# nyenyu12/BioInformatics-project-for-Shotgun-Metagenomics-Pseudo-alignment-shotgun-

Hardware: AMD Instinct MI355X
Metric: reads/sec pseudo-aligned (k=31, 150bp) at 1/2/4/8 GPUs; % HBM roofline (higher is better)
Workload: dtype u8

## Files before the change

bioinformatics-project-for-shotgun-metagenomics-pseudo-alignment-shotgun-_amd/csrc/pa_align.hip:

```cpp
#include <hip/hip_runtime.h>

#include <algorithm>
#include <cstdio>
#include <cstdlib>
#include <cstring>
#include <type_traits>
#include <vector>

#include "pa_device.h"
#include "pa_internal.h"

using namespace pad;

namespace {

constexpr int kBlock = 256;
constexpr int kWaves = kBlock / 64;
constexpr uint32_t kSegMaxWaves = 16384;
constexpr uint32_t kSegSlackWaves = 8192, kSegSlackChunks = 5;
constexpr uint64_t kSegSlack = 64ull * kSegSlackChunks * kSegSlackWaves;
constexpr uint32_t kLdsGenomeCap = 2048;

enum : uint32_t { F_MRQ = 1, F_MKQ = 2, F_MG = 4 };

// ... 15 lines not shown
    uint64_t nb_base1, nb_split;
    const uint32_t *nbbig_ld;
    uint64_t nbbig_mask;
    int nb_spec;
    const uint32_t *tile_nbbig;
    const uint4 *tile_nbm;
    int mg_nb;
    const uint32_t *gblk;
    const uint64_t *bloom;
    const uint64_t *tile_rcp;
    const uint32_t *mm_bits;
    uint32_t mm_lg;
    const uint32_t *tile_rcnb;
    uint32_t bloom_lg;
    int walk_rounds;
    int tpos_local;
    uint32_t lane_maxpend;
    int lane_noanchor;
    int dbg_mode;
    const uint8_t *seq;
    const uint8_t *qual;
    const uint64_t *off;
    uint64_t n;
    uint64_t base;
    pa::DevParams prm;
    unsigned long long *stats;
    unsigned long long *uniq;
    unsigned long long *amb;
    unsigned long long *first;
    uint32_t *queue;
    unsigned long long *qcount;
    unsigned long long *deferred_total;
    uint32_t *queue_hard;
    unsigned long long *queue_hard_count;
    uint32_t *queue_na;
    unsigned long long *queue_na_count;
    uint64_t *queue_na_keys;
    uint32_t *queue_rc;
    uint64_t *queue_rc_anc;
    unsigned long long *queue_rc_count;
    uint32_t *queue_na2;
    unsigned long long *queue_na2_count;
    uint64_t na_min;
    uint32_t na_seg;
    uint32_t *seg_cnt;
    uint32_t nseg;
    uint64_t seg_cap;
    uint64_t queue_cap;
    uint32_t *lane_next;
    const uint4 *qmask;
    const uint8_t *qdrop;
    const uint32_t *rlist;
    const unsigned long long *rlist_count;
    unsigned long long *dbg;
    uint8_t *as_type;
    uint32_t *as_len, *as_g, *as_qf, *as_hr;
};

__device__ __forceinline__ uint64_t first_key(uint64_t read, uint32_t rank) { return (read << 20) | rank; }


struct WgCounters {
    uint32_t *uniq;
    uint32_t *amb;
    unsigned long long *first;
    bool lds;
};

__device__ __forceinline__ void count_genome(const AlignArgs &a, const WgCounters &c, uint32_t g, bool unique,
                                             uint32_t times, uint64_t key) {
    if (c.lds) {
        atomicAdd(unique ? &c.uniq[g] : &c.amb[g], times);
        if (key < c.first[g]) atomicMin(&c.first[g], (unsigned long long)key);
    } else {
        atomicAdd(unique ? &a.uniq[g] : &a.amb[g], (unsigned long long)times);
        atomicMin(&a.first[g], (unsigned long long)key);
    }
}

#include "pa_fast.h"

constexpr int kQmDwords = 44;
template <int KQ>
__device__ __forceinline__ void quality_read(const uint8_t *__restrict__ qual, uint64_t o, uint32_t len, int k,
                                             uint32_t T, int64_t mrq, uint32_t flags, uint4 &mask, uint8_t &drop) {
    typedef uint32_t u32x4_a4 __attribute__((ext_vector_type(4), aligned(4)));
    const u32x4_a4 *sp = (const u32x4_a4 *)(qual + (o & ~3ull));
    const uint32_t sb = 8 * (uint32_t)(o & 3);
    uint32_t dw[kQmDwords + 4];
#pragma unroll
    for (int c = 0; c < (kQmDwords + 4) / 4; c++) {
        const u32x4_a4 v = sp[c];
        dw[4 * c] = v.x, dw[4 * c + 1] = v.y, dw[4 * c + 2] = v.z, dw[4 * c + 3] = v.w;
    }
    uint32_t rd[kQmDwords];
#pragma unroll
    for (int j = 0; j < kQmDwords; j++) rd[j] = __builtin_amdgcn_alignbit(dw[j + 1], dw[j], sb);
    const uint32_t nfull = len >> 2, pmask = (len & 3) ? (1u << (8 * (len & 3))) - 1 : 0u;
    uint32_t run_tot = 0, total = 0, part = 0;
#pragma unroll
    for (int j = 0; j < kQmDwords; j++) {
        const bool at = (uint32_t)j == nfull;
        total = at ? run_tot : total;
        part = at ? rd[j] : part;
        run_tot = __builtin_amdgcn_sad_u8(rd[j], 0u, run_tot);
    }
// ... 470 lines not shown
                    const uint32_t i = atomicAdd(&n_rank, 1u);
                    if (i < kRankLds) rank_key[i] = ld_agent(&ws.g_specmin[g]);
                }
                __syncthreads();
                for (uint32_t t = threadIdx.x; t < nt; t += kBlock) {
                    const uint32_t g = ws.touched[t];
                    if (ld_agent(&ws.g_spec[g]) == 0) continue;
                    const uint32_t mw = ld_agent(&ws.g_specmin[g]);
                    uint32_t rank = 0;
                    if (nspec <= kRankLds) {
                        for (uint32_t u = 0; u < nspec; u++) rank += rank_key[u] < mw;
                    } else {
                        for (uint32_t u = 0; u < nt; u++) {
                            const uint32_t h = ws.touched[u];
                            if (ld_agent(&ws.g_spec[h]) > 0 && ld_agent(&ws.g_specmin[h]) < mw) rank++;
                        }
                    }
                    if (x.detail == 2) x.lists[x.list_off[r] + rank] = g;
                    if (!x.detail) {
                        atomicAdd(&a.amb[g], 1ull);
                        atomicMin(&a.first[g], (unsigned long long)first_key(read_idx, rank));
                    }
                }
            }
            __syncthreads();
            for (uint32_t t = threadIdx.x; t < nt; t += kBlock) {
                const uint32_t g = ws.touched[t];
                st_agent(&ws.g_spec[g], 0u);
                st_agent(&ws.g_specmin[g], NONE);
                st_agent(&ws.g_tot[g], 0u);
                st_agent(&ws.g_totmin[g], NONE);
            }
            __syncthreads();
            if (threadIdx.x == 0) n_touched = n_cls = 0;
            __syncthreads();
        }
        if (threadIdx.x == 0) {
            if (x.detail) {
                x.type_out[r] = type;
                x.qf_out[r] = qf;
                x.hr_out[r] = hr;
                x.len_out[r] = list_len;
            } else {
                atomicAdd(&a.stats[type == PA_UNMAPPED ? 2 : (type == PA_UNIQUELY_MAPPED ? 0 : 1)], 1ull);
                if (has_mkq && qf) atomicAdd(&a.stats[4], (unsigned long long)qf);
                if (has_mg && hr) atomicAdd(&a.stats[5], (unsigned long long)hr);
            }
        }
        __syncthreads();
    }
}


size_t fast_lds_bytes(uint32_t G, int wpl, bool need_q) {
    size_t cnt = G <= kLdsGenomeCap ? (((size_t)((G + 1) & ~1u) * 16 + 15) / 16 * 16) : 0;
    size_t wl = wpl == 1 ? fast_wave_bytes<1>(need_q) : wpl == 2 ? fast_wave_bytes<2>(need_q) : fast_wave_bytes<4>(need_q);
    return cnt + kWaves * wl;
}

const char *env(const char *name) { return std::getenv(name); }
bool env_is(const char *name, char c) { const char *e = env(name); return e && e[0] == c; }
uint64_t env_u64(const char *name, uint64_t unset) { const char *e = env(name); return e ? std::strtoull(e, nullptr, 10) : unset; }
int env_int(const char *name, int unset) { const char *e = env(name); return e ? std::atoi(e) : unset; }
int env_01(const char *name) { const char *e = env(name); return e ? e[0] == '1' : -1; }

struct Switches {
    bool no_qelide = env("PA_NO_QELIDE");
    bool no_lane = env_is("PA_NO_LANE", '1');
    uint64_t lane_grid = env_u64("PA_LANE_GRID", ~0ull);
    uint32_t lane_maxpend = (uint32_t)env_int("PA_LANE_MAXPEND", 96);
    int lane_noanchor = env_01("PA_LANE_NOANCHOR");
    uint64_t na_min = env_u64("PA_NA_MIN", 32768);
    bool na_seg = !env_is("PA_NA_SEG", '0');
    bool na_rcwalk = !env_is("PA_NA_RCWALK", '0');
    bool na_rcnb = !env_is("PA_NA_RCNB", '0');
    bool mm_bits = !env_is("PA_MM_BITS", '0');
    bool no_nbbig = env("PA_NO_NBBIG");
    bool no_nbm = env("PA_NO_NBM");
    bool no_mgnb = env("PA_NO_MGNB");
    int walk_rounds = env_int("PA_WALK_ROUNDS", 1);
    int dbg_mode = env_int("PA_DBG_MODE", 0);
};

template <int N> using int_c = std::integral_constant<int, N>;

template <int N0, int... Ns, class F>
auto with_int(int n, F &&f) {
    if constexpr (sizeof...(Ns) == 0) return f(int_c<N0>{});
    else return n == N0 ? f(int_c<N0>{}) : with_int<Ns...>(n, f);
}

template <class F>
auto with_filters(uint32_t flags, F &&f) {
    const auto with_mg = [&](auto need_q, auto win_q) {
        return (flags & F_MG) ? f(need_q, win_q, std::true_type{}) : f(need_q, win_q, std::false_type{});
    };
    if (flags & F_MKQ) return with_mg(std::true_type{}, std::true_type{});
    if (flags & F_MRQ) return with_mg(std::true_type{}, std::false_type{});
    return with_mg(std::false_type{}, std::false_type{});
}

template <bool WIN_Q, class F>
auto with_shape(int nw, bool nm4, F &&f) {
    return with_int<3, 2, 1>(nw, [&](auto w) {
        if constexpr (!WIN_Q && w() == 1)
            if (nm4) return f(int_c<4>{}, w);
        return f(int_c<2>{}, w);
    });
}

using AlignKernel = void (*)(AlignArgs);
pa_status resident_grid(AlignKernel kern, int block, size_t shm, uint64_t want, unsigned &grid) {
    if (shm > 64 * 1024) PA_HIP(hipFuncSetAttribute((const void *)kern, hipFuncAttributeMaxDynamicSharedMemorySize, (int)shm));
    int per_cu = 0, dev = 0, cus = 256;
    PA_HIP(hipOccupancyMaxActiveBlocksPerMultiprocessor(&per_cu, kern, block, shm));
    PA_HIP(hipGetDevice(&dev));
    PA_HIP(hipDeviceGetAttribute(&cus, hipDeviceAttributeMultiprocessorCount, dev));
    const uint64_t resident = (uint64_t)std::max(1, per_cu) * (uint64_t)cus;
    grid = (unsigned)std::max<uint64_t>(1, std::min<uint64_t>(want, resident));
    return PA_OK;
}

struct KernelTimer {
    pa_index *idx;
    hipStream_t st;
    int slot;
    hipEvent_t e0 = nullptr;
    KernelTimer(pa_index *i, hipStream_t s, int sl) : idx(i), st(s), slot(sl) {
        if (idx && idx->profile && hipEventCreate(&e0) == hipSuccess) hipEventRecord(e0, st);
    }
    ~KernelTimer() {
        hipEvent_t e1 = nullptr;
        if (e0 && hipEventCreate(&e1) == hipSuccess && hipEventRecord(e1, st) == hipSuccess)
            idx->kev.push_back({slot, e0, e1});
        else if (e0)
            hipEventDestroy(e0);
    }
};

pa_status launch_timed(pa_index *prof, int slot, AlignKernel kern, unsigned grid, size_t shm, hipStream_t st,
                       const AlignArgs &a) {
    KernelTimer kt(prof, st, slot);
    hipLaunchKernelGGL(kern, dim3(grid), dim3(kBlock), shm, st, a);
    PA_HIP(hipGetLastError());
    return PA_OK;
}

pa_status launch_wave(const AlignArgs &a, pa_index *prof, int nw, int wpl, hipStream_t st) {
    const size_t shm = fast_lds_bytes(a.G, wpl, (a.prm.flags & (F_MRQ | F_MKQ)) != 0);
    const bool dense = a.G <= 64;
    const AlignKernel kern = with_int<1, 2, 3, 4>(nw, [&](auto w) {
        constexpr int NW = w();
        return with_int<1, 2, 4>(wpl, [&](auto l) -> AlignKernel {
            return dense ? k_align_fast<NW, l(), true> : k_align_fast<NW, l(), false>;
        });
    });
    unsigned grid = 0;
    PA_TRY(resident_grid(kern, kBlock, shm, (a.n + kWaves - 1) / kWaves, grid));
    return launch_timed(prof, PA_PROF_WAVE, kern, grid, shm, st, a);
}

constexpr uint64_t kRcnbMinReads = 32768;
struct LaneKernels { AlignKernel lane, rc, na; };
template <bool AS>
pa_status launch_lane(const AlignArgs &a0, const Switches &sw, hipStream_t st, pa_index *prof, bool long_reads, int nw) {
    const bool win_q = (a0.prm.flags & F_MKQ) != 0;
    const bool mg = (a0.prm.flags & F_MG) != 0;
    const bool nm4 = long_reads && !win_q && nw == 1;
    AlignArgs a = a0;
    const size_t shm = lane_lds_bytes(a.G, nm4 ? 4 : 2, lane_sched(win_q, mg, nm4 ? 4 : 2, nw));
    const LaneKernels kern = with_filters(a.prm.flags, [&](auto nq, auto wq, auto g) {
        constexpr bool NEED_Q = nq(), WIN_Q = wq(), MG = g();
        return LaneKernels{
            with_shape<WIN_Q>(nw, nm4, [](auto nm, auto w) -> AlignKernel { return k_align_lane<NEED_Q, WIN_Q, MG, nm(), w(), AS>; }),
            k_align_lane_rc<NEED_Q, WIN_Q, MG, AS>,
            with_int<3, 2, 1>(nw, [](auto w) -> AlignKernel {
                if constexpr (w() == 1) return k_align_lane_na<NEED_Q, WIN_Q, MG, AS>;
                else return k_align_lane_naw<NEED_Q, WIN_Q, MG, w(), AS>;
            })};
    });
    const uint64_t want = (a.n + kBlock - 1) / kBlock;
    unsigned grid = 0;
    PA_TRY(resident_grid(kern.lane, kBlock, shm, want, grid));
    grid = (unsigned)std::max<uint64_t>(1, std::min<uint64_t>(grid, sw.lane_grid));
    const uint64_t waves = (uint64_t)grid * kWaves, chunks = (a.n + 63) / 64;
    a.nseg = (uint32_t)waves;
    a.seg_cap = 64 * ((chunks + waves - 1) / waves + kLaneClaimHeld);
    a.na_seg = a.queue_na && a.queue_na_keys && a.seg_cnt && !nm4 && nw == 1 && waves <= kSegMaxWaves &&
               waves * a.seg_cap <= a.queue_cap && sw.na_seg;
    PA_TRY(launch_timed(prof, PA_PROF_LANE, kern.lane, grid, shm, st, a));
    if (!a.queue_na) return PA_OK;
    AlignArgs b = a;
    if (prof && prof->rcnb_pending && a.queue_na_keys) {
        unsigned long long c = 0;
        PA_HIP(hipMemcpyAsync(&c, a.queue_na_count, 8, hipMemcpyDeviceToHost, st));
        PA_HIP(hipStreamSynchronize(st));
        if (c >= std::max<uint64_t>(kRcnbMinReads, a.n / 64)) {
            PA_TRY(pa::index_build_rcnb(prof, st));
            if (sw.na_rcnb) b.tile_rcnb = prof->tile_rcnb;
        } else if (++prof->rcnb_checks >= 2) {
            prof->rcnb_pending = 0;
        }
    }
    if (a.queue_na_keys) {
        const unsigned sgrid = a.na_seg ? (a.nseg + kSegGroup - 1) / kSegGroup
                                        : (unsigned)std::max<uint64_t>(1, std::min<uint64_t>(
                                              (a.n + kBlock * 4 - 1) / (kBlock * 4), 8192));
        PA_TRY(launch_timed(prof, PA_PROF_RC_SEEDS, k_rc_seeds, sgrid, 0, st, b));
        PA_TRY(resident_grid(kern.rc, kBlock, 0, want, grid));
        PA_TRY(launch_timed(prof, PA_PROF_LANE_RC, kern.rc, grid, 0, st, b));
        b.queue_na = a.queue_na2;
// ... 358 lines not shown
    DevParams p;
    PA_TRY(effective_params(r, p_in, p, st, sw));
    AlignArgs a = make_args(idx, r, p, base, sw);
    const uint32_t G = idx->n_genomes;
    a.stats = (unsigned long long *)(as ? as->scratch : acc->sum_block);
    a.uniq = a.stats + 6;
    a.amb = a.uniq + G;
    a.first = as ? a.amb + G : (unsigned long long *)acc->min_block;
    if (as) a.as_type = as->type, a.as_len = as->len, a.as_g = as->g, a.as_qf = as->qf, a.as_hr = as->hr;
    a.queue = idx->queue;
    a.qcount = (unsigned long long *)idx->counters;
    a.deferred_total = (unsigned long long *)idx->counters + 1;
    a.dbg = (unsigned long long *)idx->counters + 4;
    PA_HIP(hipMemsetAsync(idx->counters, 0, 8, st));
#ifdef PA_STATS
    PA_HIP(hipMemsetAsync(a.dbg, 0, 36 * 8, st));
#endif
    const DetailOut out{as ? as->type : nullptr, as ? as->qf : nullptr, as ? as->hr : nullptr, as ? as->len : nullptr,
                        nullptr, nullptr};
    ExactArgs x;
    unsigned egrid = 0;
    PA_TRY(exact_args(idx, r, a, as ? &out : nullptr, x, egrid));
    const bool fast_ok = idx->k > 0 && idx->nw <= 4 && idx->n_kmers > 0;
    const bool lane_ok = fast_ok && idx->nw <= 3 && a.tile_n > 0 && a.tile_lw && !sw.no_lane && (!as || as->lane);
    if (queued) *queued = as && lane_ok;
    if (as ? lane_ok : fast_ok) {
        hipEvent_t e0 = nullptr, e1 = nullptr;
        if (idx->profile) {
            PA_HIP(hipEventCreate(&e0));
            PA_HIP(hipEventCreate(&e1));
            PA_HIP(hipEventRecord(e0, st));
        }
        if (lane_ok) {
            PA_TRY(mg_planes(idx, a, sw, st));
            a.queue_hard = idx->queue_hard;
            a.queue_hard_count = (unsigned long long *)idx->counters + 3;
            PA_HIP(hipMemsetAsync(idx->counters + 3, 0, 8, st));
            PA_TRY(quality_prepass(idx, r, a, st));
            PA_TRY(seedless_queues(idx, a, sw, st));
            const bool long_reads = r->max_len > (uint32_t)kLaneMaxLen ||
                                    (r->max_len >= idx->k && r->max_len - idx->k + 1 > (uint32_t)kLaneMaxW);
            PA_TRY(as ? launch_lane<true>(a, sw, st, idx, long_reads, idx->nw)
                      : launch_lane<false>(a, sw, st, idx, long_reads, idx->nw));
            a.rlist = idx->queue_hard;
            a.rlist_count = a.queue_hard_count;
        }
        if (as) {
            a.queue = idx->queue_hard;
            a.qcount = a.queue_hard_count;
            a.deferred_total = nullptr;
        } else {
            const uint32_t wmax = r->max_len >= idx->k ? (uint32_t)(r->max_len - idx->k + 1) : 0;
            const int wpl = wmax <= 64 ? 1 : wmax <= 128 ? 2 : 4;
            PA_TRY(launch_wave(a, idx, idx->nw, wpl, st));
        }
        if (idx->profile) {
            PA_HIP(hipEventRecord(e1, st));
            idx->ev_start.push_back(e0);
            idx->ev_stop.push_back(e1);
        }
        x.a = a;
        x.use_queue = 1;
    }
    PA_TRY(launch_exact(idx, idx->nw, x, egrid, st));
#ifdef PA_STATS
    PA_TRY(print_stats(idx, r, st));
#endif
    return PA_OK;
}

pa_status align(pa_index *idx, const pa_reads *r, const DevParams &p, uint64_t base, pa_result *acc,
                hipStream_t st) {
    return align_pass(idx, r, p, base, acc, nullptr, nullptr, st);
}

pa_status assign_classify(pa_index *idx, const pa_reads *r, const DevParams &p, const AssignBufs &as, bool *queued,
                          hipStream_t st) {
    return align_pass(idx, r, p, 0, nullptr, &as, queued, st);
}

pa_status assign_lists(pa_index *idx, const pa_reads *r, const DevParams &p_in, const AssignBufs &as, bool queued,
                       const uint64_t *d_off, uint32_t *d_lists, hipStream_t st) {
    if (r->n == 0) return PA_OK;
    const Switches sw;
    DevParams p;
    PA_TRY(effective_params(r, p_in, p, st, sw));
    AlignArgs a = make_args(idx, r, p, 0, sw);
    a.queue = idx->queue_hard;
    a.qcount = (unsigned long long *)idx->counters + 3;
    const DetailOut out{as.type, as.qf, as.hr, as.len, d_off, d_lists};
    ExactArgs x;
    unsigned egrid = 0;
    PA_TRY(exact_args(idx, r, a, &out, x, egrid));
    x.use_queue = queued ? 1 : 0;
    return launch_exact(idx, idx->nw, x, egrid, st);
}

pa_status detail_pass_device(pa_index *idx, const pa_reads *r, const DevParams &p, uint8_t *d_type, uint32_t *d_qf,
                             uint32_t *d_hr, uint32_t *d_len, const uint64_t *d_off, uint32_t *d_lists,
                             hipStream_t st) {
    if (r->n == 0) return PA_OK;
    const DetailOut out{d_type, d_qf, d_hr, d_len, d_off, d_lists};
    ExactArgs x;
    unsigned egrid = 0;
    PA_TRY(exact_args(idx, r, make_args(idx, r, p, 0, Switches{}), &out, x, egrid));
    return launch_exact(nullptr, idx->nw, x, egrid, st);
}
// ... 54 lines not shown
```

bioinformatics-project-for-shotgun-metagenomics-pseudo-alignment-shotgun-_amd/csrc/pa_fast.h:

```cpp

#ifndef PA_HS_PER_WPL
#define PA_HS_PER_WPL 128
#endif
template <int WPL>
struct FastCfg {
    static constexpr int HS = PA_HS_PER_WPL * WPL;
    static constexpr int E = HS / 64;
    static constexpr int LCAP = 64 * WPL + 64;
    static constexpr int NDW = (LCAP + 8 + 255) / 256;
    static constexpr int PW = NDW * 8 + 2;
    static constexpr int BW = NDW * 4 + 2;
};

template <int WPL>
struct __align__(16) WaveLds {
    using C = FastCfg<WPL>;
    uint64_t packed[C::PW];
    uint64_t diff[C::PW];
    uint64_t poison[C::BW];
    uint64_t hA_key[C::HS];
    uint32_t hA_v[C::HS];
    uint32_t hA_v2[C::HS];
    uint32_t hB_key[C::HS];
    uint32_t hB_cnt[C::HS];
    uint32_t hB_min[C::HS];
    uint32_t gcnt[64];
    uint32_t gmin[64];
};

template <int WPL>
struct __align__(16) WaveQual {
    using C = FastCfg<WPL>;
    uint32_t stage[C::NDW * 64];
    uint32_t pref[C::LCAP + 4];
};

__device__ __forceinline__ uint32_t lds_hash_slot(uint64_t key, uint32_t mask) {
    return (uint32_t)((key * 0x9E3779B97F4A7C15ull) >> 40) & mask;
}

__device__ __forceinline__ uint32_t lds_insert64(uint64_t *keys, uint32_t hs, uint64_t key) {
    uint32_t p = lds_hash_slot(key, hs - 1);
    for (;;) {
        uint64_t old = atomicCAS((unsigned long long *)&keys[p], (unsigned long long)EMPTY, (unsigned long long)key);
        if (old == EMPTY || old == key) return p;
        p = (p + 1) & (hs - 1);
    }
}

__device__ __forceinline__ uint32_t lds_insert32(uint32_t *keys, uint32_t hs, uint32_t key) {
    uint32_t p = lds_hash_slot(key, hs - 1);
    for (;;) {
        uint32_t old = atomicCAS(&keys[p], NONE, key);
        if (old == NONE || old == key) return p;
        p = (p + 1) & (hs - 1);
    }
}

__device__ __forceinline__ uint32_t lds_insert64_bounded(uint64_t *keys, uint32_t hs, uint64_t key) {
    uint32_t p = lds_hash_slot(key, hs - 1);
    for (uint32_t it = 0; it < hs; it++) {
        uint64_t old = atomicCAS((unsigned long long *)&keys[p], (unsigned long long)EMPTY, (unsigned long long)key);
        if (old == EMPTY || old == key) return p;
        p = (p + 1) & (hs - 1);
    }
    return hs;
}

template <int WPL>
__device__ __forceinline__ void load_stage(const uint8_t *base, uint64_t o, uint32_t (&d)[FastCfg<WPL>::NDW]) {
    const uint32_t *p = (const uint32_t *)(base + (o & ~3ull));
#pragma unroll
    for (int j = 0; j < FastCfg<WPL>::NDW; j++) d[j] = p[lane_id() + 64 * j];
}

enum : int { OUT_UNIQUE = 0, OUT_AMB = 1, OUT_DEFER = 2, OUT_UNMAPPED = 3, OUT_DROP = 4 };

struct ReadTotals {
    uint32_t qf = 0, hr = 0;
    uint32_t unique = 0, mapped = 0, unm = 0, drop = 0;
#ifdef PA_STATS
    uint32_t d_win = 0, d_probe = 0, d_walk = 0, d_anchor = 0;
#endif
};

__device__ __forceinline__ bool bit(uint32_t m, int i) { return (m >> i) & 1u; }

template <int WPL, typename SettledFn, typename MultiFn>
__device__ __forceinline__ int dense_core(const AlignArgs &a, const WgCounters &wc, WaveLds<WPL> &L, uint64_t r,
                                          bool has_multi, SettledFn settled, MultiFn multi) {
    const int lane = lane_id();
    const uint32_t G = a.G;
    const uint32_t cnt = L.gcnt[lane], smin = L.gmin[lane];
    const uint64_t specb = __ballot(cnt > 0);
    const uint32_t nspec = (uint32_t)__popcll(specb);
    const uint64_t read_idx = a.base + r;
    if (nspec == 0) return OUT_AMB;
    const uint64_t key = cnt > 0 ? (((uint64_t)cnt << 32) | (NONE - smin)) : 0;
    const uint64_t top = wave_max64(key);
    const int gstar = __builtin_ctzll(__ballot(key == top));
    const uint32_t topcnt = (uint32_t)(top >> 32);
    const uint32_t second = wave_max(lane == gstar ? 0u : cnt);
    const bool unique = nspec == 1 || (int64_t)topcnt >= (int64_t)second + a.prm.m;
    if (!unique) {
        uint32_t rank = 0;
        for (uint64_t m = specb; m; m &= m - 1) rank += __builtin_amdgcn_readlane(smin, __builtin_ctzll(m)) < smin;
        if (cnt > 0) count_genome(a, wc, lane, false, 1, first_key(read_idx, rank));
        return OUT_AMB;
    }
    const uint32_t nmulti = (a.prm.p < 0 || !has_multi || settled(gstar)) ? 0u : multi();
    if (nmulti == 0) {
        if (lane == 0) count_genome(a, wc, gstar, true, 1, first_key(read_idx, 0));
        return OUT_UNIQUE;
    }
    uint32_t t = cnt, tmin = cnt > 0 ? smin : NONE;
    for (uint32_t j = 0; j < nmulti; j++) {
        const uint64_t msk = L.hA_key[j];
        if ((msk >> lane) & 1) {
            t += L.hA_v[j];
            tmin = min(tmin, L.hA_v2[j]);
        }
    }
    const uint32_t tstar = __builtin_amdgcn_readlane(t, gstar);
    const uint32_t maxtot = wave_max(t);
    if ((int64_t)maxtot - (int64_t)tstar > a.prm.p) {
        const bool q = (uint32_t)lane < G && t >= tstar;
        const uint64_t qb = __ballot(q);
        const uint64_t me = ((uint64_t)tmin << 32) | (uint32_t)lane;
        uint32_t rank = 1;
        for (uint64_t m = qb; m; m &= m - 1) {
            const int s = __builtin_ctzll(m);
            rank += ((((uint64_t)__builtin_amdgcn_readlane(tmin, s)) << 32) | (uint32_t)s) < me;
        }
        if (q) count_genome(a, wc, lane, false, lane == gstar ? 2 : 1, first_key(read_idx, lane == gstar ? 0 : rank));
        return OUT_AMB;
    }
    if (lane == 0) count_genome(a, wc, gstar, true, 1, first_key(read_idx, 0));
    return OUT_UNIQUE;
}

template <int WPL>
__device__ __forceinline__ uint32_t dense_multi_list(const AlignArgs &a, WaveLds<WPL> &L) {
    using C = FastCfg<WPL>;
    const int lane = lane_id();
    uint32_t nmulti = 0;
#pragma unroll
    for (int e = 0; e < C::E; e++) {
        const int i = lane + 64 * e;
        const uint32_t c = L.hB_key[i];
        const uint32_t is_multi = (c != NONE && c >= a.G) ? 1u : 0u;
        const uint64_t bm = __ballot(is_multi);
        if (is_multi) {
            const uint32_t at = nmulti + lanes_below(bm);
            L.hA_key[at] = a.class_mask[c - a.G];
            L.hA_v[at] = L.hB_cnt[i];
            L.hA_v2[at] = L.hB_min[i];
        }
        nmulti += (uint32_t)__popcll(bm);
    }
    wave_sync();
    return nmulti;
}

template <int WPL>
__device__ __forceinline__ int decide_dense(const AlignArgs &a, const WgCounters &wc, WaveLds<WPL> &L, uint64_t r) {
    using C = FastCfg<WPL>;
    const int lane = lane_id();
#pragma unroll
    for (int e = 0; e < C::E; e++) {
        const int i = lane + 64 * e;
        const uint32_t c = L.hB_key[i];
        if (c < a.G) {
            L.gcnt[c] = L.hB_cnt[i];
            L.gmin[c] = L.hB_min[i];
        }
    }
    const uint32_t nmulti = dense_multi_list<WPL>(a, L);
    return dense_core<WPL>(a, wc, L, r, nmulti > 0, [](int) { return false; }, [&]() { return nmulti; });
}

template <int WPL>
__device__ __forceinline__ int decide_hash(const AlignArgs &a, const WgCounters &wc, WaveLds<WPL> &L, uint64_t r) {
    using C = FastCfg<WPL>;
    const int lane = lane_id();
    const uint32_t G = a.G;
    uint32_t specm = 0, multim = 0;
    uint32_t nspec = 0, nmulti = 0;
    uint64_t top_l = 0;
#pragma unroll
    for (int e = 0; e < C::E; e++) {
        const int i = lane + 64 * e;
        const uint32_t c = L.hB_key[i];
        const uint32_t sp = c < G ? 1u : 0u, mu = (c != NONE && c >= G) ? 1u : 0u;
        specm |= sp << e;
        multim |= mu << e;
        nspec += (uint32_t)__popcll(__ballot(sp));
        nmulti += (uint32_t)__popcll(__ballot(mu));
        if (sp) {
            const uint64_t t = ((uint64_t)L.hB_cnt[i] << 48) | ((uint64_t)(0xFFFFu - L.hB_min[i]) << 32) | c;
            top_l = t > top_l ? t : top_l;
        }
    }
    const uint64_t read_idx = a.base + r;
    if (nspec == 0) return OUT_AMB;
    const uint64_t top = wave_max64(top_l);
    const uint32_t gstar = (uint32_t)top, topcnt = (uint32_t)(top >> 48);
    uint32_t sec_l = 0;
#pragma unroll
    for (int e = 0; e < C::E; e++)
        if (bit(specm, e) && L.hB_key[lane + 64 * e] != gstar) sec_l = max(sec_l, L.hB_cnt[lane + 64 * e]);
    const uint32_t second = wave_max(sec_l);
    const bool unique = nspec == 1 || (int64_t)topcnt >= (int64_t)second + a.prm.m;
    if (!unique) {
        uint32_t mymin[C::E], rank[C::E];
#pragma unroll
        for (int e = 0; e < C::E; e++) {
            mymin[e] = bit(specm, e) ? L.hB_min[lane + 64 * e] : NONE;
            rank[e] = 0;
        }
#pragma unroll
        for (int f = 0; f < C::E; f++) {
            for (uint64_t m = __ballot(bit(specm, f)); m; m &= m - 1) {
                const uint32_t other = L.hB_min[__builtin_ctzll(m) + 64 * f];
#pragma unroll
                for (int e = 0; e < C::E; e++) rank[e] += other < mymin[e];
            }
        }
#pragma unroll
        for (int e = 0; e < C::E; e++)
            if (bit(specm, e)) count_genome(a, wc, L.hB_key[lane + 64 * e], false, 1, first_key(read_idx, rank[e]));
        return OUT_AMB;
    }
    if (a.prm.p < 0 || nmulti == 0) {
        if (lane == 0) count_genome(a, wc, gstar, true, 1, first_key(read_idx, 0));
        return OUT_UNIQUE;
// ... 65 lines not shown
        uint64_t me[C::E];
        uint32_t rank[C::E];
#pragma unroll
        for (int e = 0; e < C::E; e++) {
            const int i = lane + 64 * e;
            qm |= (L.hA_key[i] != EMPTY && L.hA_v[i] >= tstar ? 1u : 0u) << e;
            me[e] = ((uint64_t)L.hA_v2[i] << 32) | (uint32_t)L.hA_key[i];
            rank[e] = 1;
        }
#pragma unroll
        for (int f = 0; f < C::E; f++) {
            for (uint64_t m = __ballot(bit(qm, f)); m; m &= m - 1) {
                const uint32_t i = __builtin_ctzll(m) + 64 * f;
                const uint64_t other = ((uint64_t)L.hA_v2[i] << 32) | (uint32_t)L.hA_key[i];
#pragma unroll
                for (int e = 0; e < C::E; e++) rank[e] += other < me[e];
            }
        }
#pragma unroll
        for (int e = 0; e < C::E; e++) {
            if (!bit(qm, e)) continue;
            const uint32_t g = (uint32_t)me[e];
            if (g == gstar)
                count_genome(a, wc, g, false, 2, first_key(read_idx, 0));
            else
                count_genome(a, wc, g, false, 1, first_key(read_idx, rank[e]));
        }
        return OUT_AMB;
    }
    if (lane == 0) count_genome(a, wc, gstar, true, 1, first_key(read_idx, 0));
    return OUT_UNIQUE;
}

template <int NW, int WPL>
struct Windows {
    Key<NW> key[WPL];
    uint64_t slot[NW == 1 ? 1 : WPL];
    uint32_t cls[WPL];
    uint32_t pend, inc, qf, hr;
    uint32_t walk;
    uint32_t ga;
};

__device__ __forceinline__ uint32_t swar_codes(uint32_t x) { return ((x >> 1) ^ (x >> 2)) & 0x03030303u; }
__device__ __forceinline__ uint32_t swar_bad_bytes(uint32_t x, uint32_t codes) {
    const uint32_t d = x ^ __builtin_amdgcn_perm(0u, 0x54474341u, codes);
    return ((d & 0x7F7F7F7Fu) + 0x7F7F7F7Fu | d) & 0x80808080u;
}
__device__ __forceinline__ uint32_t swar_pack_byte(uint32_t codes) {
    return (codes * ((1u << 30) | (1u << 20) | (1u << 10) | 1u)) >> 24;
}

template <int NW, int WPL, bool DENSE>
__device__ __forceinline__ bool prep_read(const AlignArgs &a, WaveLds<WPL> &L, WaveQual<WPL> *Q, bool need_q,
                                          uint32_t shift, uint32_t len, const uint32_t (&sd)[FastCfg<WPL>::NDW],
                                          const uint32_t (&qd)[FastCfg<WPL>::NDW], Windows<NW, WPL> &S,
                                          ReadTotals &tot) {
    using C = FastCfg<WPL>;
    const int lane = lane_id();
    const int k = a.k;
    const uint32_t flags = a.prm.flags;
    const uint32_t W = (len >= (uint32_t)k) ? len - k + 1 : 0;
    wave_sync();
    if (need_q) {
#pragma unroll
        for (int j = 0; j < C::NDW; j++) Q->stage[lane + 64 * j] = qd[j];
    }
    if (DENSE && NW == 1) {
        L.gcnt[lane] = 0;
        L.gmin[lane] = NONE;
#pragma unroll
        for (int e = 0; e < C::E; e++) L.hA_key[C::E * lane + e] = EMPTY;
    }
    uint32_t badany = 0;
    uint8_t *pk8 = (uint8_t *)L.packed;
#pragma unroll
    for (int j = 0; j < C::NDW; j++) {
        const uint32_t x = sd[j];
        const uint32_t cd = swar_codes(x);
        const uint32_t p0 = 4u * (lane + 64 * j);
        uint32_t bad = swar_bad_bytes(x, cd);
        const uint32_t lo = shift > p0 ? shift - p0 : 0u, hi = shift + len > p0 ? shift + len - p0 : 0u;
        const uint32_t inr = (hi >= 4 ? 0xFFFFFFFFu : ((1u << (8 * hi)) - 1)) & (lo >= 4 ? 0u : (0xFFFFFFFFu << (8 * lo)));
        badany |= bad & inr;
        pk8[(lane + 64 * j) ^ 7] = (uint8_t)swar_pack_byte(cd);
    }
    if (lane < 2) L.packed[C::PW - 2 + lane] = 0;
    const bool any_bad = __ballot(badany != 0) != 0;
    if (any_bad) {
        if (lane < C::BW) L.poison[lane] = 0;
        wave_sync();
#pragma unroll
        for (int j = 0; j < C::NDW; j++) {
            const uint32_t x = sd[j];
            const uint32_t p0 = 4u * (lane + 64 * j);
            const uint32_t lo = shift > p0 ? shift - p0 : 0u, hi = shift + len > p0 ? shift + len - p0 : 0u;
            const uint32_t inr =
                (hi >= 4 ? 0xFFFFFFFFu : ((1u << (8 * hi)) - 1)) & (lo >= 4 ? 0u : (0xFFFFFFFFu << (8 * lo)));
            const uint32_t bad = swar_bad_bytes(x, swar_codes(x)) & inr;
            const uint32_t nib = ((bad >> 7) & 1u) | ((bad >> 14) & 2u) | ((bad >> 21) & 4u) | ((bad >> 28) & 8u);
            if (nib) atomicOr((uint32_t *)L.poison + (p0 >> 5), nib << (p0 & 31));
        }
    }
    wave_sync();
    if (need_q) {
        const uint8_t *qb = (const uint8_t *)Q->stage + shift;
        uint32_t carry = 0;
        for (uint32_t c0 = 0; c0 < len; c0 += 64) {
            const uint32_t i = c0 + lane;
            const uint32_t s = wave_incl_scan(i < len ? (uint32_t)qb[i] : 0u) + carry;
            Q->pref[i + 1] = s;
            carry = __shfl(s, 63);
        }
        if (lane == 0) Q->pref[0] = 0;
        wave_sync();
        if ((flags & F_MRQ) && (int64_t)Q->pref[len] < (int64_t)a.prm.mrq * (int64_t)len) {
            return false;
        }
    }
    const int64_t mkq_k = (int64_t)a.prm.mkq * k;
    S.pend = S.inc = S.qf = S.hr = S.walk = 0;
    S.ga = NONE;
#pragma unroll
    for (int j = 0; j < WPL; j++) {
        const uint32_t w = lane + 64 * j;
        uint32_t ok = w < W ? 1u : 0u;
        if (ok && (flags & F_MKQ) && (int64_t)(Q->pref[w + k] - Q->pref[w]) < mkq_k) {
            S.qf++;
            ok = 0;
        }
        if (ok && any_bad && window_any(L.poison, w + shift, k)) ok = 0;
        S.key[j] = extract_key<NW>(L.packed, w + shift, k);
        S.pend |= ok << j;
    }
    return true;
}

template <int NW, int WPL>
__device__ __forceinline__ void resolve_read(const AlignArgs &a, WaveLds<WPL> &L, uint32_t shift,
                                             Windows<NW, WPL> &S, ReadTotals &tot) {
    using C = FastCfg<WPL>;
    const int lane = lane_id();
    const int k = a.k;
    const uint32_t flags = a.prm.flags;
    const Slot<NW> *table = (const Slot<NW> *)a.table;
    auto resolve = [&](int j, uint32_t c) {
        c = cls_of(c);
        S.cls[j] = c;
        if ((flags & F_MG) && (int64_t)class_size_of(c, a.G, a.class_genomes) > (int64_t)a.prm.mg)
            S.hr++;
        else
            S.inc |= 1u << j;
    };
    auto probe = [&](uint32_t m, uint32_t (&tp)[WPL]) -> uint32_t {
        uint32_t found = 0;
#ifdef PA_STATS
        tot.d_probe += __popc(m);
#endif
        uint64_t pos[WPL];
#pragma unroll
        for (int j = 0; j < WPL; j++)
            if (bit(m, j)) pos[j] = home_of<NW>(S.key[j], key_hash(S.key[j]), a.home);
        while (__ballot(m != 0)) {
            Slot<NW> s[WPL];
#pragma unroll
            for (int j = 0; j < WPL; j++)
                if (bit(m, j)) s[j] = table[pos[j]];
#pragma unroll
            for (int j = 0; j < WPL; j++) {
                if (!bit(m, j)) continue;
                if (s[j].key[0] == EMPTY) {
                    m &= ~(1u << j);
                    continue;
                }
                bool eq = true;
#pragma unroll
                for (int t = 0; t < NW; t++) eq &= (s[j].key[t] == S.key[j].w[t]);
                if (eq) {
                    m &= ~(1u << j);
                    found |= 1u << j;
                    tp[j] = s[j].tpos;
                    if constexpr (NW > 1) S.slot[j] = pos[j];
                    resolve(j, s[j].cls);
                } else if (probe_past<NW>(s[j], S.key[j], pos[j], a.home)) {
                    m &= ~(1u << j);
                } else {
                    pos[j] = (pos[j] + 1 == a.cap) ? 0 : pos[j] + 1;
                }
            }
        }
        return found;
    };
// ... 84 lines not shown
                if (bit(S.pend, j) && t < a.tile_n) {
                    const uint32_t v = a.tile_cls[t];
                    tc[j] = v == NONE ? NONE : (v & ~PA_TILE_REP);
                }
            }
            wave_sync();
#pragma unroll
            for (int j = 0; j < WPL; j++)
                if (tc[j] != NONE && (get64(L.diff, 2 * (lane + 64 * j + shift)) >> sh) == 0) {
#ifdef PA_STATS
                    tot.d_walk++;
#endif
                    S.pend &= ~(1u << j);
                    const uint64_t t = (uint64_t)(A + lane + 64 * j);
                    if (t >= gs && t < ge) S.walk |= 1u << j;
                    resolve(j, tc[j]);
                }
        }
        uint32_t *list = L.hA_v, *res = L.hA_v2;
        uint32_t npend = 0;
#pragma unroll
        for (int j = 0; j < WPL; j++) {
            const uint64_t b = __ballot(bit(S.pend, j));
            if (bit(S.pend, j)) list[npend + lanes_below(b)] = lane + 64 * j;
            npend += (uint32_t)__popcll(b);
        }
        if (npend == 0) return;
        wave_sync();
#ifdef PA_STATS
        tot.d_probe += lane < (int)npend ? 1u : 0u;
#endif
        for (uint32_t base = 0; base < npend; base += 64) {
            const bool act = base + lane < npend;
            const uint32_t w = act ? list[base + lane] : 0u;
            uint32_t c = NONE, t = NONE;
            probe_one(act, w, c, t);
            if (act) res[w] = c;
        }
        wave_sync();
#pragma unroll
        for (int j = 0; j < WPL; j++)
            if (bit(S.pend, j)) {
                const uint32_t c = res[lane + 64 * j];
                if (c != NONE) resolve(j, c);
            }
        S.pend = 0;
        return;
    }
    probe(S.pend, tp);
    S.pend = 0;
}

template <int NW, int WPL, bool DENSE>
__device__ __forceinline__ int decide_general(const AlignArgs &a, const WgCounters &wc, WaveLds<WPL> &L,
                                              const Windows<NW, WPL> &S, uint64_t r) {
    using C = FastCfg<WPL>;
    const int lane = lane_id();
    const uint32_t incm = S.inc;
#pragma unroll
    for (int e = 0; e < C::E; e++) {
        const int i = lane + 64 * e;
        L.hA_key[i] = EMPTY;
        L.hA_v[i] = NONE;
        L.hB_key[i] = NONE;
        L.hB_cnt[i] = 0;
        L.hB_min[i] = NONE;
    }
    if (DENSE) {
        L.gcnt[lane] = 0;
        L.gmin[lane] = NONE;
    }
    wave_sync();
    uint32_t hp[WPL];
#pragma unroll
    for (int j = 0; j < WPL; j++)
        if (bit(incm, j)) {
            uint64_t id;
            if constexpr (NW == 1)
                id = S.key[j].w[0];
            else
                id = S.slot[j];
            hp[j] = lds_insert64(L.hA_key, C::HS, id);
            atomicMin(&L.hA_v[hp[j]], (uint32_t)(lane + 64 * j));
        }
    wave_sync();
#pragma unroll
    for (int j = 0; j < WPL; j++)
        if (bit(incm, j) && L.hA_v[hp[j]] == (uint32_t)(lane + 64 * j)) {
            const uint32_t p = lds_insert32(L.hB_key, C::HS, S.cls[j]);
            atomicAdd(&L.hB_cnt[p], 1u);
            atomicMin(&L.hB_min[p], (uint32_t)(lane + 64 * j));
        }
    wave_sync();
    if (DENSE)
        return decide_dense<WPL>(a, wc, L, r);
    else
        return decide_hash<WPL>(a, wc, L, r);
}

template <int WPL>
__device__ __forceinline__ int decide_dense_fast(const AlignArgs &a, const WgCounters &wc, WaveLds<WPL> &L,
                                                 const Windows<1, WPL> &S, uint64_t r) {
    using C = FastCfg<WPL>;
    const int lane = lane_id();
    const uint32_t incm = S.inc;
    uint32_t firstm = 0, multim = 0;
#pragma unroll
    for (int j = 0; j < WPL; j++)
        if (bit(incm, j)) {
            const uint64_t key = S.key[j].w[0];
            uint32_t p = lds_hash_slot(key, C::HS - 1);
            for (;;) {
                const uint64_t old = atomicCAS((unsigned long long *)&L.hA_key[p], (unsigned long long)EMPTY,
                                               (unsigned long long)key);
                if (old == EMPTY) firstm |= 1u << j;
                if (old == EMPTY || old == key) break;
                p = (p + 1) & (C::HS - 1);
            }
            const uint32_t c = S.cls[j];
            if (c < a.G) {
                if (bit(firstm, j)) atomicAdd(&L.gcnt[c], 1u);
                atomicMin(&L.gmin[c], (uint32_t)(lane + 64 * j));
            } else {
                multim |= 1u << j;
            }
        }
    const bool has_multi = __ballot(multim != 0) != 0;
    wave_sync();
#ifdef PA_STATS
    if (a.dbg_mode == 4) return OUT_AMB;
#endif
    auto settled = [&](int gstar) -> bool {
        uint32_t lack = 0;
#pragma unroll
        for (int j = 0; j < WPL; j++)
            if (bit(firstm, j)) {
                const uint32_t c = S.cls[j];
                bool has;
                if (c < a.G)
                    has = c == (uint32_t)gstar;
                else if (bit(S.walk, j) && S.ga == (uint32_t)gstar)
                    has = true;
                else
                    has = (a.class_mask[c - a.G] >> gstar) & 1;
                lack += has ? 0u : 1u;
            }
        return (int64_t)wave_sum(lack) <= (int64_t)a.prm.p;
    };
    return dense_core<WPL>(a, wc, L, r, has_multi, settled, [&]() -> uint32_t {
#pragma unroll
        for (int e = 0; e < C::E; e++) {
            const int i = lane + 64 * e;
            L.hB_key[i] = NONE;
            L.hB_cnt[i] = 0;
            L.hB_min[i] = NONE;
        }
        wave_sync();
#pragma unroll
        for (int j = 0; j < WPL; j++)
            if (bit(multim, j)) {
                const uint32_t p = lds_insert32(L.hB_key, C::HS, S.cls[j]);
                if (bit(firstm, j)) atomicAdd(&L.hB_cnt[p], 1u);
                atomicMin(&L.hB_min[p], (uint32_t)(lane + 64 * j));
            }
        wave_sync();
        return dense_multi_list<WPL>(a, L);
    });
}

template <int NW, int WPL, bool DENSE>
__device__ __forceinline__ int classify_read(const AlignArgs &a, const WgCounters &wc, WaveLds<WPL> &L,
                                             WaveQual<WPL> *Q, bool need_q, uint64_t r, uint32_t shift, uint32_t len,
                                             const uint32_t (&sd)[FastCfg<WPL>::NDW],
                                             const uint32_t (&qd)[FastCfg<WPL>::NDW], Windows<NW, WPL> &S,
                                             ReadTotals &tot) {
    if (!prep_read<NW, WPL, DENSE>(a, L, Q, need_q, shift, len, sd, qd, S, tot)) return OUT_DROP;
#ifdef PA_STATS
    tot.d_win += __popc(S.pend);
    if (a.dbg_mode == 2) return OUT_UNMAPPED;
#endif
    resolve_read<NW, WPL>(a, L, shift, S, tot);
#ifdef PA_STATS
    if (a.dbg_mode == 3) return OUT_UNMAPPED;
#endif
    if (!__ballot(S.inc != 0)) return OUT_UNMAPPED;
    if constexpr (DENSE && NW == 1)
        return decide_dense_fast<WPL>(a, wc, L, S, r);
    else
        return decide_general<NW, WPL, DENSE>(a, wc, L, S, r);
}

template <int NW, int WPL, bool DENSE>
__device__ __forceinline__ void fast_read(const AlignArgs &a, const WgCounters &wc, WaveLds<WPL> &L,
                                          WaveQual<WPL> *Q, bool need_q, uint64_t r, uint32_t shift, uint32_t len,
                                          const uint32_t (&sd)[FastCfg<WPL>::NDW],
                                          const uint32_t (&qd)[FastCfg<WPL>::NDW], ReadTotals &tot) {
    Windows<NW, WPL> S;
    const int out = classify_read<NW, WPL, DENSE>(a, wc, L, Q, need_q, r, shift, len, sd, qd, S, tot);
    const bool counted = out != OUT_DROP && out != OUT_DEFER;
    tot.qf += counted ? S.qf : 0u;
    tot.hr += counted ? S.hr : 0u;
    tot.unique += out == OUT_UNIQUE ? 1u : 0u;
    tot.mapped += (out == OUT_UNIQUE || out == OUT_AMB) ? 1u : 0u;
    tot.unm += out == OUT_UNMAPPED ? 1u : 0u;
    tot.drop += out == OUT_DROP ? 1u : 0u;
}

#ifndef PA_FAST_MIN_WAVES
#define PA_FAST_MIN_WAVES 1
#endif
template <int NW, int WPL, bool DENSE>
__global__ __launch_bounds__(kBlock, PA_FAST_MIN_WAVES) void k_align_fast(AlignArgs a) {
    using C = FastCfg<WPL>;
    extern __shared__ __align__(16) unsigned char smem[];
    const int lane = lane_id();
    const int wid = threadIdx.x >> 6;
    const uint32_t G = a.G;
    const bool need_q = a.prm.flags & (F_MRQ | F_MKQ);

    WgCounters wc;
    wc.lds = G <= kLdsGenomeCap;
    const uint32_t Gl = wc.lds ? ((G + 1) & ~1u) : 0;
    wc.first = (unsigned long long *)smem;
    wc.uniq = (uint32_t *)(wc.first + Gl);
    wc.amb = wc.uniq + Gl;
    unsigned char *wave_base = smem + ((size_t)Gl * 16 + 15) / 16 * 16;
    WaveLds<WPL> &L = ((WaveLds<WPL> *)wave_base)[wid];
    WaveQual<WPL> *Q = ((WaveQual<WPL> *)(wave_base + kWaves * sizeof(WaveLds<WPL>))) + wid;
    for (uint32_t i = threadIdx.x; i < Gl; i += kBlock) {
        wc.first[i] = (unsigned long long)PA_NO_FIRST_KEY;
        wc.uniq[i] = 0;
        wc.amb[i] = 0;
    }
    __syncthreads();

    const uint64_t nq = a.rlist ? (uint64_t)*a.rlist_count : a.n;
    const uint64_t nw = (uint64_t)gridDim.x * kWaves, gw = (uint64_t)blockIdx.x * kWaves + wid;
    const uint64_t qb = nq * gw / nw, qe = nq * (gw + 1) / nw;
    ReadTotals tot;
    if (qb < qe) {
        uint64_t r = a.rlist ? a.rlist[qb] : qb;
        uint64_t o_cur = a.off[r], o_end = a.off[r + 1];
        uint32_t sd[C::NDW], qd[C::NDW];
        load_stage<WPL>(a.seq, o_cur, sd);
        if (need_q) load_stage<WPL>(a.qual, o_cur, qd);
        for (uint64_t q = qb; q < qe; q++) {
            uint64_t r_n = 0, o_n = 0, e_n = 0;
            uint32_t sn[C::NDW], qn[C::NDW];
            if (q + 1 < qe) {
                r_n = a.rlist ? a.rlist[q + 1] : q + 1;
                o_n = a.off[r_n];
                e_n = a.off[r_n + 1];
                load_stage<WPL>(a.seq, o_n, sn);
                if (need_q) load_stage<WPL>(a.qual, o_n, qn);
            }
            const uint32_t len = (uint32_t)(o_end - o_cur);
            const uint32_t W = (len >= (uint32_t)a.k) ? len - a.k + 1 : 0;
            if (W > 64u * WPL || len > (uint32_t)(C::LCAP - 8)) {
                if (lane == 0) a.queue[atomicAdd(a.qcount, 1ull)] = (uint32_t)r;
            } else {
                fast_read<NW, WPL, DENSE>(a, wc, L, Q, need_q, r, (uint32_t)(o_cur & 3), len, sd, qd, tot);
            }
            r = r_n;
            o_cur = o_n;
            o_end = e_n;
#pragma unroll
            for (int j = 0; j < C::NDW; j++) {
                sd[j] = sn[j];
                qd[j] = qn[j];
            }
        }
    }
    const uint32_t qf_w = wave_sum(tot.qf), hr_w = wave_sum(tot.hr);
    const bool has_mkq = a.prm.flags & F_MKQ, has_mg = a.prm.flags & F_MG;
#ifdef PA_STATS
    {
        const uint32_t s0 = wave_sum(tot.d_win), s1 = wave_sum(tot.d_probe), s2 = wave_sum(tot.d_walk),
                       s3 = wave_sum(tot.d_anchor);
        if (lane == 0) {
            atomicAdd(&a.dbg[0], (unsigned long long)s0);
            atomicAdd(&a.dbg[1], (unsigned long long)s1);
            atomicAdd(&a.dbg[2], (unsigned long long)s2);
            atomicAdd(&a.dbg[3], (unsigned long long)s3);
        }
    }
#endif
    if (lane == 0) {
        if (tot.unique) atomicAdd(&a.stats[0], (unsigned long long)tot.unique);
        if (tot.mapped > tot.unique) atomicAdd(&a.stats[1], (unsigned long long)(tot.mapped - tot.unique));
        if (tot.unm) atomicAdd(&a.stats[2], (unsigned long long)tot.unm);
        if (tot.drop) atomicAdd(&a.stats[3], (unsigned long long)tot.drop);
        if (qf_w && has_mkq) atomicAdd(&a.stats[4], (unsigned long long)qf_w);
        if (hr_w && has_mg) atomicAdd(&a.stats[5], (unsigned long long)hr_w);
    }
    if (wc.lds) {
        __syncthreads();
        for (uint32_t g = threadIdx.x; g < G; g += kBlock) {
            if (wc.uniq[g]) atomicAdd(&a.uniq[g], (unsigned long long)wc.uniq[g]);
            if (wc.amb[g]) atomicAdd(&a.amb[g], (unsigned long long)wc.amb[g]);
            if (wc.first[g] != (unsigned long long)PA_NO_FIRST_KEY) atomicMin(&a.first[g], wc.first[g]);
        }
    }
}

template <int WPL>
constexpr size_t fast_wave_bytes(bool need_q) {
    return sizeof(WaveLds<WPL>) + (need_q ? sizeof(WaveQual<WPL>) : 0);
}
```

Before: 4.577 billion.

## Trim per-wave LDS for sparse kernels and raise hash-path occupancy

Moves the 64-entry gcnt/gmin dense scratch into a base struct that exists only for the dense kernel variant, so the hash (sparse) variant uses less LDS per wave. When an rlist is present, the host checks whether dropping the per-block genome counters from LDS (falling back to global atomics) would allow more resident blocks, and drops them if so. It also raises the launch-bounds minimum waves for the NW=1, WPL=2, sparse kernel to push register allocation lower, and adds an env override for the wave grid size. The intent is higher occupancy and better latency hiding for memory-bound hash lookups. The cost is more global atomic traffic when counters leave LDS, and possible register spills from the tighter launch bound.

```diff
diff --git a/bioinformatics-project-for-shotgun-metagenomics-pseudo-alignment-shotgun-_amd/csrc/pa_align.hip b/bioinformatics-project-for-shotgun-metagenomics-pseudo-alignment-shotgun-_amd/csrc/pa_align.hip
--- a/bioinformatics-project-for-shotgun-metagenomics-pseudo-alignment-shotgun-_amd/csrc/pa_align.hip
+++ b/bioinformatics-project-for-shotgun-metagenomics-pseudo-alignment-shotgun-_amd/csrc/pa_align.hip
@@ -91,6 +91,7 @@
     const uint8_t *qdrop;
     const uint32_t *rlist;
     const unsigned long long *rlist_count;
+    int wave_lds_cnt;
     unsigned long long *dbg;
     uint8_t *as_type;
     uint32_t *as_len, *as_g, *as_qf, *as_hr;
@@ -667,9 +668,10 @@
 }
 
 
-size_t fast_lds_bytes(uint32_t G, int wpl, bool need_q) {
-    size_t cnt = G <= kLdsGenomeCap ? (((size_t)((G + 1) & ~1u) * 16 + 15) / 16 * 16) : 0;
-    size_t wl = wpl == 1 ? fast_wave_bytes<1>(need_q) : wpl == 2 ? fast_wave_bytes<2>(need_q) : fast_wave_bytes<4>(need_q);
+size_t fast_lds_bytes(uint32_t G, int wpl, bool dense, bool need_q, bool lds_cnt) {
+    size_t cnt = lds_cnt ? (((size_t)((G + 1) & ~1u) * 16 + 15) / 16 * 16) : 0;
+    size_t wl = wpl == 1 ? fast_wave_bytes<1>(dense, need_q) : wpl == 2 ? fast_wave_bytes<2>(dense, need_q)
+                                                                         : fast_wave_bytes<4>(dense, need_q);
     return cnt + kWaves * wl;
 }
 
@@ -683,6 +685,7 @@
     bool no_qelide = env("PA_NO_QELIDE");
     bool no_lane = env_is("PA_NO_LANE", '1');
     uint64_t lane_grid = env_u64("PA_LANE_GRID", ~0ull);
+    uint64_t wave_grid = env_u64("PA_WAVE_GRID", ~0ull);
     uint32_t lane_maxpend = (uint32_t)env_int("PA_LANE_MAXPEND", 96);
     int lane_noanchor = env_01("PA_LANE_NOANCHOR");
     uint64_t na_min = env_u64("PA_NA_MIN", 32768);
@@ -725,10 +728,14 @@
 }
 
 using AlignKernel = void (*)(AlignArgs);
+pa_status resident_per_cu(AlignKernel kern, int block, size_t shm, int &per_cu) {
+    if (shm > 64 * 1024) PA_HIP(hipFuncSetAttribute((const void *)kern, hipFuncAttributeMaxDynamicSharedMemorySize, (int)shm));
+    PA_HIP(hipOccupancyMaxActiveBlocksPerMultiprocessor(&per_cu, kern, block, shm));
+    return PA_OK;
+}
 pa_status resident_grid(AlignKernel kern, int block, size_t shm, uint64_t want, unsigned &grid) {
-    if (shm > 64 * 1024) PA_HIP(hipFuncSetAttribute((const void *)kern, hipFuncAttributeMaxDynamicSharedMemorySize, (int)shm));
     int per_cu = 0, dev = 0, cus = 256;
-    PA_HIP(hipOccupancyMaxActiveBlocksPerMultiprocessor(&per_cu, kern, block, shm));
+    PA_TRY(resident_per_cu(kern, block, shm, per_cu));
     PA_HIP(hipGetDevice(&dev));
     PA_HIP(hipDeviceGetAttribute(&cus, hipDeviceAttributeMultiprocessorCount, dev));
     const uint64_t resident = (uint64_t)std::max(1, per_cu) * (uint64_t)cus;
@@ -761,17 +768,27 @@
     return PA_OK;
 }
 
-pa_status launch_wave(const AlignArgs &a, pa_index *prof, int nw, int wpl, hipStream_t st) {
-    const size_t shm = fast_lds_bytes(a.G, wpl, (a.prm.flags & (F_MRQ | F_MKQ)) != 0);
+pa_status launch_wave(const AlignArgs &a0, const Switches &sw, pa_index *prof, int nw, int wpl, hipStream_t st) {
+    AlignArgs a = a0;
     const bool dense = a.G <= 64;
+    const bool need_q = (a.prm.flags & (F_MRQ | F_MKQ)) != 0;
     const AlignKernel kern = with_int<1, 2, 3, 4>(nw, [&](auto w) {
         constexpr int NW = w();
         return with_int<1, 2, 4>(wpl, [&](auto l) -> AlignKernel {
             return dense ? k_align_fast<NW, l(), true> : k_align_fast<NW, l(), false>;
         });
     });
+    a.wave_lds_cnt = a.G <= kLdsGenomeCap;
+    if (a.wave_lds_cnt && PA_FAST_REM_GLOBAL && a.rlist) {
+        int with = 0, without = 0;
+        PA_TRY(resident_per_cu(kern, kBlock, fast_lds_bytes(a.G, wpl, dense, need_q, true), with));
+        PA_TRY(resident_per_cu(kern, kBlock, fast_lds_bytes(a.G, wpl, dense, need_q, false), without));
+        if (without > with) a.wave_lds_cnt = 0;
+    }
+    const size_t shm = fast_lds_bytes(a.G, wpl, dense, need_q, a.wave_lds_cnt);
     unsigned grid = 0;
     PA_TRY(resident_grid(kern, kBlock, shm, (a.n + kWaves - 1) / kWaves, grid));
+    grid = (unsigned)std::max<uint64_t>(1, std::min<uint64_t>(grid, sw.wave_grid));
     return launch_timed(prof, PA_PROF_WAVE, kern, grid, shm, st, a);
 }
 
@@ -1236,7 +1253,7 @@
         } else {
             const uint32_t wmax = r->max_len >= idx->k ? (uint32_t)(r->max_len - idx->k + 1) : 0;
             const int wpl = wmax <= 64 ? 1 : wmax <= 128 ? 2 : 4;
-            PA_TRY(launch_wave(a, idx, idx->nw, wpl, st));
+            PA_TRY(launch_wave(a, sw, idx, idx->nw, wpl, st));
         }
         if (idx->profile) {
             PA_HIP(hipEventRecord(e1, st));
diff --git a/bioinformatics-project-for-shotgun-metagenomics-pseudo-alignment-shotgun-_amd/csrc/pa_fast.h b/bioinformatics-project-for-shotgun-metagenomics-pseudo-alignment-shotgun-_amd/csrc/pa_fast.h
--- a/bioinformatics-project-for-shotgun-metagenomics-pseudo-alignment-shotgun-_amd/csrc/pa_fast.h
+++ b/bioinformatics-project-for-shotgun-metagenomics-pseudo-alignment-shotgun-_amd/csrc/pa_fast.h
@@ -1,6 +1,12 @@
 
 #ifndef PA_HS_PER_WPL
 #define PA_HS_PER_WPL 128
+#endif
+#ifndef PA_FAST_REM_GLOBAL
+#define PA_FAST_REM_GLOBAL 1
+#endif
+#ifndef PA_FAST_HASH_WAVES
+#define PA_FAST_HASH_WAVES 5
 #endif
 template <int WPL>
 struct FastCfg {
@@ -12,8 +18,16 @@
     static constexpr int BW = NDW * 4 + 2;
 };
 
-template <int WPL>
-struct __align__(16) WaveLds {
+template <bool DENSE>
+struct DenseLds {
+    uint32_t gcnt[64];
+    uint32_t gmin[64];
+};
+template <>
+struct DenseLds<false> {};
+
+template <int WPL, bool DENSE>
+struct __align__(16) WaveLds : DenseLds<DENSE> {
     using C = FastCfg<WPL>;
     uint64_t packed[C::PW];
     uint64_t diff[C::PW];
@@ -24,8 +38,6 @@
     uint32_t hB_key[C::HS];
     uint32_t hB_cnt[C::HS];
     uint32_t hB_min[C::HS];
-    uint32_t gcnt[64];
-    uint32_t gmin[64];
 };
 
 template <int WPL>
@@ -87,7 +99,7 @@
 __device__ __forceinline__ bool bit(uint32_t m, int i) { return (m >> i) & 1u; }
 
 template <int WPL, typename SettledFn, typename MultiFn>
-__device__ __forceinline__ int dense_core(const AlignArgs &a, const WgCounters &wc, WaveLds<WPL> &L, uint64_t r,
+__device__ __forceinline__ int dense_core(const AlignArgs &a, const WgCounters &wc, WaveLds<WPL, true> &L, uint64_t r,
                                           bool has_multi, SettledFn settled, MultiFn multi) {
     const int lane = lane_id();
     const uint32_t G = a.G;
@@ -140,7 +152,7 @@
 }
 
 template <int WPL>
-__device__ __forceinline__ uint32_t dense_multi_list(const AlignArgs &a, WaveLds<WPL> &L) {
+__device__ __forceinline__ uint32_t dense_multi_list(const AlignArgs &a, WaveLds<WPL, true> &L) {
     using C = FastCfg<WPL>;
     const int lane = lane_id();
     uint32_t nmulti = 0;
@@ -163,7 +175,7 @@
 }
 
 template <int WPL>
-__device__ __forceinline__ int decide_dense(const AlignArgs &a, const WgCounters &wc, WaveLds<WPL> &L, uint64_t r) {
+__device__ __forceinline__ int decide_dense(const AlignArgs &a, const WgCounters &wc, WaveLds<WPL, true> &L, uint64_t r) {
     using C = FastCfg<WPL>;
     const int lane = lane_id();
 #pragma unroll
@@ -180,7 +192,7 @@
 }
 
 template <int WPL>
-__device__ __forceinline__ int decide_hash(const AlignArgs &a, const WgCounters &wc, WaveLds<WPL> &L, uint64_t r) {
+__device__ __forceinline__ int decide_hash(const AlignArgs &a, const WgCounters &wc, WaveLds<WPL, false> &L, uint64_t r) {
     using C = FastCfg<WPL>;
     const int lane = lane_id();
     const uint32_t G = a.G;
@@ -352,7 +364,7 @@
 }
 
 template <int NW, int WPL, bool DENSE>
-__device__ __forceinline__ bool prep_read(const AlignArgs &a, WaveLds<WPL> &L, WaveQual<WPL> *Q, bool need_q,
+__device__ __forceinline__ bool prep_read(const AlignArgs &a, WaveLds<WPL, DENSE> &L, WaveQual<WPL> *Q, bool need_q,
                                           uint32_t shift, uint32_t len, const uint32_t (&sd)[FastCfg<WPL>::NDW],
                                           const uint32_t (&qd)[FastCfg<WPL>::NDW], Windows<NW, WPL> &S,
                                           ReadTotals &tot) {
@@ -366,7 +378,7 @@
 #pragma unroll
         for (int j = 0; j < C::NDW; j++) Q->stage[lane + 64 * j] = qd[j];
     }
-    if (DENSE && NW == 1) {
+    if constexpr (DENSE && NW == 1) {
         L.gcnt[lane] = 0;
         L.gmin[lane] = NONE;
 #pragma unroll
@@ -436,8 +448,8 @@
     return true;
 }
 
-template <int NW, int WPL>
-__device__ __forceinline__ void resolve_read(const AlignArgs &a, WaveLds<WPL> &L, uint32_t shift,
+template <int NW, int WPL, bool DENSE>
+__device__ __forceinline__ void resolve_read(const AlignArgs &a, WaveLds<WPL, DENSE> &L, uint32_t shift,
                                              Windows<NW, WPL> &S, ReadTotals &tot) {
     using C = FastCfg<WPL>;
     const int lane = lane_id();
@@ -628,7 +640,7 @@
 }
 
 template <int NW, int WPL, bool DENSE>
-__device__ __forceinline__ int decide_general(const AlignArgs &a, const WgCounters &wc, WaveLds<WPL> &L,
+__device__ __forceinline__ int decide_general(const AlignArgs &a, const WgCounters &wc, WaveLds<WPL, DENSE> &L,
                                               const Windows<NW, WPL> &S, uint64_t r) {
     using C = FastCfg<WPL>;
     const int lane = lane_id();
@@ -642,7 +654,7 @@
         L.hB_cnt[i] = 0;
         L.hB_min[i] = NONE;
     }
-    if (DENSE) {
+    if constexpr (DENSE) {
         L.gcnt[lane] = 0;
         L.gmin[lane] = NONE;
     }
@@ -668,14 +680,14 @@
             atomicMin(&L.hB_min[p], (uint32_t)(lane + 64 * j));
         }
     wave_sync();
-    if (DENSE)
+    if constexpr (DENSE)
         return decide_dense<WPL>(a, wc, L, r);
     else
         return decide_hash<WPL>(a, wc, L, r);
 }
 
 template <int WPL>
-__device__ __forceinline__ int decide_dense_fast(const AlignArgs &a, const WgCounters &wc, WaveLds<WPL> &L,
+__device__ __forceinline__ int decide_dense_fast(const AlignArgs &a, const WgCounters &wc, WaveLds<WPL, true> &L,
                                                  const Windows<1, WPL> &S, uint64_t r) {
     using C = FastCfg<WPL>;
     const int lane = lane_id();
@@ -745,7 +757,7 @@
 }
 
 template <int NW, int WPL, bool DENSE>
-__device__ __forceinline__ int classify_read(const AlignArgs &a, const WgCounters &wc, WaveLds<WPL> &L,
+__device__ __forceinline__ int classify_read(const AlignArgs &a, const WgCounters &wc, WaveLds<WPL, DENSE> &L,
                                              WaveQual<WPL> *Q, bool need_q, uint64_t r, uint32_t shift, uint32_t len,
                                              const uint32_t (&sd)[FastCfg<WPL>::NDW],
                                              const uint32_t (&qd)[FastCfg<WPL>::NDW], Windows<NW, WPL> &S,
@@ -755,7 +767,7 @@
     tot.d_win += __popc(S.pend);
     if (a.dbg_mode == 2) return OUT_UNMAPPED;
 #endif
-    resolve_read<NW, WPL>(a, L, shift, S, tot);
+    resolve_read<NW, WPL, DENSE>(a, L, shift, S, tot);
 #ifdef PA_STATS
     if (a.dbg_mode == 3) return OUT_UNMAPPED;
 #endif
@@ -767,7 +779,7 @@
 }
 
 template <int NW, int WPL, bool DENSE>
-__device__ __forceinline__ void fast_read(const AlignArgs &a, const WgCounters &wc, WaveLds<WPL> &L,
+__device__ __forceinline__ void fast_read(const AlignArgs &a, const WgCounters &wc, WaveLds<WPL, DENSE> &L,
                                           WaveQual<WPL> *Q, bool need_q, uint64_t r, uint32_t shift, uint32_t len,
                                           const uint32_t (&sd)[FastCfg<WPL>::NDW],
                                           const uint32_t (&qd)[FastCfg<WPL>::NDW], ReadTotals &tot) {
@@ -785,8 +797,11 @@
 #ifndef PA_FAST_MIN_WAVES
 #define PA_FAST_MIN_WAVES 1
 #endif
+constexpr int fast_min_waves(int nw, int wpl, bool dense) {
+    return nw == 1 && wpl == 2 && !dense ? PA_FAST_HASH_WAVES : PA_FAST_MIN_WAVES;
+}
 template <int NW, int WPL, bool DENSE>
-__global__ __launch_bounds__(kBlock, PA_FAST_MIN_WAVES) void k_align_fast(AlignArgs a) {
+__global__ __launch_bounds__(kBlock, fast_min_waves(NW, WPL, DENSE)) void k_align_fast(AlignArgs a) {
     using C = FastCfg<WPL>;
     extern __shared__ __align__(16) unsigned char smem[];
     const int lane = lane_id();
@@ -795,14 +810,14 @@
     const bool need_q = a.prm.flags & (F_MRQ | F_MKQ);
 
     WgCounters wc;
-    wc.lds = G <= kLdsGenomeCap;
+    wc.lds = a.wave_lds_cnt;
     const uint32_t Gl = wc.lds ? ((G + 1) & ~1u) : 0;
     wc.first = (unsigned long long *)smem;
     wc.uniq = (uint32_t *)(wc.first + Gl);
     wc.amb = wc.uniq + Gl;
     unsigned char *wave_base = smem + ((size_t)Gl * 16 + 15) / 16 * 16;
-    WaveLds<WPL> &L = ((WaveLds<WPL> *)wave_base)[wid];
-    WaveQual<WPL> *Q = ((WaveQual<WPL> *)(wave_base + kWaves * sizeof(WaveLds<WPL>))) + wid;
+    WaveLds<WPL, DENSE> &L = ((WaveLds<WPL, DENSE> *)wave_base)[wid];
+    WaveQual<WPL> *Q = ((WaveQual<WPL> *)(wave_base + kWaves * sizeof(WaveLds<WPL, DENSE>))) + wid;
     for (uint32_t i = threadIdx.x; i < Gl; i += kBlock) {
         wc.first[i] = (unsigned long long)PA_NO_FIRST_KEY;
         wc.uniq[i] = 0;
@@ -880,6 +895,6 @@
 }
 
 template <int WPL>
-constexpr size_t fast_wave_bytes(bool need_q) {
-    return sizeof(WaveLds<WPL>) + (need_q ? sizeof(WaveQual<WPL>) : 0);
-}
+constexpr size_t fast_wave_bytes(bool dense, bool need_q) {
+    return (dense ? sizeof(WaveLds<WPL, true>) : sizeof(WaveLds<WPL, false>)) + (need_q ? sizeof(WaveQual<WPL>) : 0);
+}
```

Result: no change. 4.598 billion, median of 6 (+0.5%).
